# hibikid39/ndt_slam

Measured on AMD Instinct MI355X. Metric: scan-matches/sec (10k-pt scan vs 1M-pt NDT map), higher is better.
Workload: dtype f64

## Files before the change

ndt_slam_amd/csrc/ndt_map_build.hip.h:

```cpp


__device__ __forceinline__ unsigned f2ord(float f) {
  unsigned u = __float_as_uint(f);
  return (u & 0x80000000u) ? ~u : (u | 0x80000000u);
}
__host__ __device__ inline float ord2f(unsigned u) {
  u = (u & 0x80000000u) ? (u & 0x7fffffffu) : ~u;
  float f;
#if defined(__HIP_DEVICE_COMPILE__)
  f = __uint_as_float(u);
#else
  memcpy(&f, &u, 4);
#endif
  return f;
}

__global__ void __launch_bounds__(256)
map_minmax_kernel(const float *__restrict__ xy, size_t stride, size_t n, unsigned *__restrict__ bounds,
                  unsigned *__restrict__ out) {
  __shared__ float sh[4][4];
  float mnx = FLT_MAX, mny = FLT_MAX, mxx = -FLT_MAX, mxy = -FLT_MAX;
  const size_t step = (size_t)gridDim.x * blockDim.x;
  for (size_t i0 = blockIdx.x * (size_t)blockDim.x + threadIdx.x; i0 < n; i0 += 16 * step) {
    float2 p[16];
// ... 195 lines not shown
    for (int r = 0; r < 4; ++r) p[r] = e < n[r] ? load_pt(xy, stride, (size_t)mine[r]) : make_float2(0.f, 0.f);
#pragma unroll
    for (int r = 0; r < 4; ++r) {
      if (e >= n[r]) continue;
      int rank = 0;
      for (int j = 0; j < n[r]; j += 4) {
        const ndt_i4v q = *(const NDT_GLOBAL ndt_i4v_u *)(perm + s0[r] + j);
        rank += (q.x < mine[r]) ? 1 : 0;
        rank += (j + 1 < n[r] && q.y < mine[r]) ? 1 : 0;
        rank += (j + 2 < n[r] && q.z < mine[r]) ? 1 : 0;
        rank += (j + 3 < n[r] && q.w < mine[r]) ? 1 : 0;
      }
      pts[s0[r] + rank] = p[r];
    }
  }
}

constexpr int kBigWavesPerBlock = 4, kBigBlocks = 4096, kBigStage = 512;
constexpr int kBigRuns = 64;
__global__ void __launch_bounds__(256)
map_order_kernel(const int *__restrict__ start, size_t ng, unsigned small_blocks, const int *__restrict__ big,
                 const int *__restrict__ nbig, int big_cap, const int *__restrict__ perm, const float *__restrict__ xy,
                 size_t stride, float2 *__restrict__ pts) {
  __shared__ int stage[kBigWavesPerBlock][kBigStage];
  __shared__ int run_first[kBigWavesPerBlock][kBigRuns], run_pos[kBigWavesPerBlock][kBigRuns + 1];
  if (blockIdx.x < small_blocks) { order_small_voxels(blockIdx.x, start, ng, perm, xy, stride, pts); return; }
  const unsigned bblock = blockIdx.x - small_blocks, bblocks = gridDim.x - small_blocks;
  const int lane = threadIdx.x & 63, wv = threadIdx.x >> 6;
  const u64 lt = (1ull << lane) - 1ull;
  const int count = min(*nbig, big_cap);
  for (int q = bblock * kBigWavesPerBlock + wv; q < count; q += bblocks * kBigWavesPerBlock) {
    const int g = big[q];
    const int s0 = start[g], n = start[g + 1] - s0;
    const bool staged = n <= kBigStage;
    int nruns = 0;
    if (staged) {
      for (int e = lane; e < n; e += 64) stage[wv][e] = perm[s0 + e];
      __builtin_amdgcn_wave_barrier();
      for (int base = 0; base < n; base += 64) {
        const int e = base + lane;
        const int idx = e < n ? stage[wv][e] : 0, prev = (e > 0 && e < n) ? stage[wv][e - 1] : -2;
        const bool head = e < n && (e == 0 || idx != prev + 1);
        const u64 hm = __ballot(head);
        if (head) {
          const int r = nruns + __builtin_popcountll(hm & lt);
          if (r < kBigRuns) { run_first[wv][r] = idx; run_pos[wv][r] = e; }
        }
        nruns += __builtin_popcountll(hm);
      }
      if (lane == 0 && nruns <= kBigRuns) run_pos[wv][nruns] = n;
      __builtin_amdgcn_wave_barrier();
    }
    if (staged && nruns <= kBigRuns) {
      int seen = 0;
      for (int base = 0; base < n; base += 64) {
        const int e = base + lane;
        const int idx = e < n ? stage[wv][e] : 0, prev = (e > 0 && e < n) ? stage[wv][e - 1] : -2;
        const bool head = e < n && (e == 0 || idx != prev + 1);
        const u64 hm = __ballot(head);
        const int myrun = seen + __builtin_popcountll(hm & (lt | (1ull << lane))) - 1;
        seen += __builtin_popcountll(hm);
        if (e >= n) continue;
        const float2 p = load_pt(xy, stride, (size_t)idx);
        const int myfirst = run_first[wv][myrun], off = e - run_pos[wv][myrun];
        int dest = 0;
        for (int r = 0; r < nruns; ++r) {
          const int f = run_first[wv][r], len = run_pos[wv][r + 1] - run_pos[wv][r];
          dest += (f < myfirst) ? len : 0;
        }
        pts[s0 + dest + off] = p;
      }
      continue;
    }
    for (int e = lane; e < n; e += 64) {
      const int mine = staged ? stage[wv][e] : perm[s0 + e];
      int rank = 0;
      if (staged) { for (int j = 0; j < n; ++j) rank += (stage[wv][j] < mine) ? 1 : 0; }
      else        { for (int j = 0; j < n; ++j) rank += (perm[s0 + j] < mine) ? 1 : 0; }
      pts[s0 + rank] = load_pt(xy, stride, (size_t)mine);
    }
  }
}

struct LeafParams { int min_pts, cov_unbiased, cov_init_identity; double eig_mult; };

__device__ int leaf_finalize(const LeafParams &L, int n, double sx, double sy, double sxx,
                             double sxy, double syy, double szz, double mean[2], double icov[3]) {
  const double dn = (double)n;
  const double mx = sx / dn, my = sy / dn;
  mean[0] = mx; mean[1] = my;
  icov[0] = icov[1] = icov[2] = 0.0;
  double cxx, cxy, cyy, czz;
  if (!L.cov_unbiased) {
    cxx = (sxx - 2.0 * (sx * mx)) / dn + mx * mx;
    cxy = (sxy - 2.0 * (sy * mx)) / dn + my * mx;
    cyy = (syy - 2.0 * (sy * my)) / dn + my * my;
    czz = szz / dn;
    const double f = (dn - 1.0) / dn;
    cxx *= f; cxy *= f; cyy *= f; czz *= f;
  } else {
    cxx = (sxx - sx * mx) / (dn - 1.0);
    cxy = (sxy - sy * mx) / (dn - 1.0);
    cyy = (syy - sy * my) / (dn - 1.0);
    czz = szz / (dn - 1.0);
  }
  const double hd = 0.5 * (cxx - cyy), tr = 0.5 * (cxx + cyy);
  const double rad = sqrt(hd * hd + cxy * cxy);
  const double l1 = tr - rad, l2 = tr + rad;
  double vx, vy;
  if (rad == 0.0) { vx = 1.0; vy = 0.0; }
  else if (hd >= 0.0) { vx = hd + rad; vy = cxy; }
  else { vx = cxy; vy = rad - hd; }
  const double vn = sqrt(vx * vx + vy * vy);
  if (vn == 0.0) { vx = 1.0; vy = 0.0; } else { vx /= vn; vy /= vn; }
  double ev0, ev1, ev2; int k0, k1, k2;
  if (czz <= l1)      { ev0 = czz; k0 = 2; ev1 = l1; k1 = 0; ev2 = l2; k2 = 1; }
  else if (czz <= l2) { ev0 = l1; k0 = 0; ev1 = czz; k1 = 2; ev2 = l2; k2 = 1; }
  else                { ev0 = l1; k0 = 0; ev1 = l2; k1 = 1; ev2 = czz; k2 = 2; }
  if (ev0 < 0 || ev1 < 0 || ev2 <= 0) return 0;
  const double thr = L.eig_mult * ev2;
  bool rebuilt = false;
  if (ev0 < thr) { ev0 = thr; if (ev1 < thr) ev1 = thr; rebuilt = true; }
  double n1 = l1, n2 = l2;
  if (k0 == 0) n1 = ev0; else if (k0 == 1) n2 = ev0;
  if (k1 == 0) n1 = ev1; else if (k1 == 1) n2 = ev1;
  if (k2 == 0) n1 = ev2; else if (k2 == 1) n2 = ev2;
  if (rebuilt) {
    cxx = n1 * (vy * vy) + n2 * (vx * vx);
    cxy = -n1 * (vx * vy) + n2 * (vx * vy);
    cyy = n1 * (vx * vx) + n2 * (vy * vy);
  }
  const double det = cxx * cyy - cxy * cxy;
  icov[0] = cyy / det; icov[1] = -cxy / det; icov[2] = cxx / det;
  for (int a = 0; a < 3; ++a)
    if (icov[a] == (double)INFINITY || icov[a] == -(double)INFINITY) return -1;
  return 1;
}

__device__ __forceinline__ int write_voxel(const GridDims &G, const LeafParams &L, size_t g, int n, float fx, float fy,
                                           double sx, double sy, double sxx, double sxy, double syy, double szz,
                                           float2 *__restrict__ cent, double *__restrict__ rec, int *__restrict__ ) {
  if (n < L.min_pts) return 0;
  const int ix = (int)(g % G.div_x), iy = (int)(g / G.div_x);
  const size_t pg = (size_t)(iy + 2) * G.gw + (ix + 2);
  double mean[2], icov[3];
  const int ok = leaf_finalize(L, n, sx, sy, sxx, sxy, syy, szz, mean, icov);
  cent[pg] = make_float2(fx / (float)n, fy / (float)n);
  double *r = rec + pg * 8;
  r[0] = mean[0]; r[1] = mean[1]; r[2] = icov[0]; r[3] = icov[1]; r[4] = icov[2];
  r[5] = __longlong_as_double((long long)(((u64)__float_as_uint(fy / (float)n) << 32) | (u64)__float_as_uint(fx / (float)n)));
  return ok > 0 ? n : -n;
}

constexpr int kFinStage = 1536;
__global__ void __launch_bounds__(256)
map_finalize_kernel(GridDims G, LeafParams L,
                          const int *__restrict__ start,
                          const float2 *__restrict__ pts, float2 *__restrict__ cent, double *__restrict__ rec,
                          int *__restrict__ npts_grid, int *__restrict__ counters ,
                          unsigned *__restrict__ occ ,
                          u64 *__restrict__ tiles, int tiles_w ) {
  __shared__ float2 lp[4][kFinStage];
  const size_t ng = (size_t)G.div_x * G.div_y;
  size_t g = blockIdx.x * (size_t)blockDim.x + threadIdx.x;
  const bool live = g < ng;
  const int lane = threadIdx.x & 63, wv = threadIdx.x >> 6;
  int s0 = 0, s1 = 0;
  if (live) { s0 = start[g]; s1 = start[g + 1]; }
  const int n = s1 - s0;
  const int a = __shfl(s0, 0);
  int b = s1;
#pragma unroll
  for (int o = 1; o < 64; o <<= 1) b = max(b, __shfl_xor(b, o));
  const int m = b - a;
  const bool in_lds = m <= kFinStage;
  if (in_lds) {
    for (int j0 = 0; j0 < m; j0 += 8 * 64) {
      float2 t[8];
#pragma unroll
      for (int u = 0; u < 8; ++u) { const int j = j0 + u * 64 + lane; t[u] = pts[a + min(j, m - 1)]; }
#pragma unroll
      for (int u = 0; u < 8; ++u) { const int j = j0 + u * 64 + lane; if (j < m) lp[wv][j] = t[u]; }
    }
    __builtin_amdgcn_wave_barrier();
  }
  int flag = 0;
  if (n > 0) {
    float fx = 0.f, fy = 0.f;
    double sx = 0, sy = 0, sxx = 0, sxy = 0, syy = 0, szz = 0;
    if (L.cov_init_identity) { sxx = 1.0; syy = 1.0; szz = 1.0; }
    if (in_lds) {
      const float2 *q = &lp[wv][s0 - a];
      for (int s = 0; s < n; ++s) {
        const float2 p = q[s];
        fx += p.x; fy += p.y;
        const double X = (double)p.x, Y = (double)p.y;
        sx += X; sy += Y;
        sxx += X * X; sxy += X * Y; syy += Y * Y;
      }
    } else {
      float2 pb[8], pn[8];
#pragma unroll
      for (int u = 0; u < 8; ++u) pb[u] = pts[min(s0 + u, s1 - 1)];
      for (int s = s0; s < s1; s += 8) {
        if (s + 8 < s1) {
#pragma unroll
          for (int u = 0; u < 8; ++u) pn[u] = pts[min(s + 8 + u, s1 - 1)];
        }
#pragma unroll
        for (int u = 0; u < 8; ++u) {
          if (s + u >= s1) break;
          const float2 p = pb[u];
          fx += p.x; fy += p.y;
          const double X = (double)p.x, Y = (double)p.y;
          sx += X; sy += Y;
          sxx += X * X; sxy += X * Y; syy += Y * Y;
        }
#pragma unroll
        for (int u = 0; u < 8; ++u) pb[u] = pn[u];
      }
    }
    flag = write_voxel(G, L, g, n, fx, fy, sx, sy, sxx, sxy, syy, szz, cent, rec, counters);
    const int vy = (int)(g / (size_t)G.div_x), vx = (int)(g - (size_t)vy * G.div_x);
    atomicOr(tiles + (size_t)((vy >> 3) + 1) * tiles_w + (vx >> 3) + 1, 1ull << (8 * (vy & 7) + (vx & 7)));
  }
  if (live) npts_grid[g] = flag;
  const u64 in_set = __ballot(flag != 0);
  if ((threadIdx.x & 63) == 0 && live) {
    occ[g >> 5] = (unsigned)in_set;
    if ((g >> 5) + 1 < (ng + 31) / 32) occ[(g >> 5) + 1] = (unsigned)(in_set >> 32);
  }
}

__global__ void fill_f2_kernel(float2 *p, size_t n, float v, u64 *tiles, size_t ntiles) {
  for (size_t i = blockIdx.x * (size_t)blockDim.x + threadIdx.x; i < n; i += (size_t)gridDim.x * blockDim.x)
    p[i] = make_float2(v, v);
  for (size_t i = blockIdx.x * (size_t)blockDim.x + threadIdx.x; i < ntiles; i += (size_t)gridDim.x * blockDim.x)
    tiles[i] = 0ull;
}
```

ndt_slam_amd/csrc/ndt_mi355x.hip:

```cpp

#include <hip/hip_runtime.h>
#include <hip/hip_ext.h>

#include <algorithm>
#include <cfloat>
#include <cmath>
#include <cstdio>
#include <cstdlib>
#include <cstring>
#include <new>
#include <string>
#include <mutex>
#include <set>
#include <utility>
#include <vector>

#include "ndt_mi355x.h"

#pragma clang fp contract(off)

namespace {

thread_local std::string g_last_error;

#include "ndt_libm_f32.hip.h"
#include "ndt_common.hip.h"
#include "ndt_point.hip.h"
#include "ndt_optimizer.hip.h"
#include "ndt_fitness.hip.h"
#include "ndt_match.hip.h"
#include "ndt_map_build.hip.h"
#include "ndt_front.hip.h"
#include "ndt_localmap.hip.h"

}


struct ndt_ctx {
  int device = 0;
  hipStream_t stream = nullptr;
  hipStream_t own_stream = nullptr;
  hipEvent_t ev0 = nullptr, ev1 = nullptr;
  hipEvent_t evm0 = nullptr, evm1 = nullptr;
  hipEvent_t evb = nullptr;
  ndt_map *pending_map = nullptr;
  hipStream_t side = nullptr;
  hipEvent_t ev_fork = nullptr, ev_join = nullptr;
  bool map_ms_pending = false;
  unsigned *h_bounds = nullptr;
  std::string err;
  float map_ms = 0.f, align_ms = 0.f;
  void *d_scan = nullptr; size_t d_scan_cap = 0;
  void *d_off = nullptr; size_t d_off_cap = 0;
  void *d_init = nullptr; size_t d_init_cap = 0;
  void *d_res = nullptr; size_t d_res_cap = 0;
  void *d_tmp = nullptr; size_t d_tmp_cap = 0;
  void *d_trace = nullptr; size_t d_trace_cap = 0;
  void *d_rows = nullptr; size_t d_rows_cap = 0;
  void *d_sorted = nullptr; size_t d_sorted_cap = 0;
  void *d_sorted_x[2] = {nullptr, nullptr}; size_t d_sorted_x_cap[2] = {0, 0};
  void *d_fit = nullptr; size_t d_fit_cap = 0;
  void *d_fit_part = nullptr; size_t d_fit_part_cap = 0;
  void *d_far = nullptr; size_t d_far_cap = 0;
  void *d_ws = nullptr; size_t d_ws_cap = 0;
  void *d_ws_x[2] = {nullptr, nullptr}; size_t d_ws_x_cap[2] = {0, 0};
  void *d_pf = nullptr; size_t d_pf_cap = 0;
  void *d_rn = nullptr; size_t d_rn_cap = 0;
  void *d_mm = nullptr; size_t d_mm_cap = 0;
  void *h_mm = nullptr; size_t h_mm_cap = 0;
  hipEvent_t ev_mm = nullptr; bool mm_pending = false;
  int num_cus = 0;
  int helpers = -1;
  int workgroups = 0;
  int inject_fault = 0;
  struct PrepSet {
    void *sorted = nullptr; size_t sorted_cap = 0;
    void *recs = nullptr; size_t recs_cap = 0;
    void *maps = nullptr; size_t maps_cap = 0;
    hipEvent_t ev0 = nullptr, ready = nullptr;
    bool valid = false, timed = false;
    const void *scans = nullptr, *offsets = nullptr, *inits = nullptr, *map = nullptr;
    int B = 0, shared_scan = 0; size_t total_points = 0;
    int min_bx = 0, min_by = 0, div_x = 0, div_y = 0; float inv_leaf = 0.f;
    long long reader = -1;
  } prep[2];
  int prep_last = 1;
  float order_ms = 0.f;
  hipEvent_t ev_scratch = nullptr; hipStream_t scratch_stream = nullptr; bool scratch_used = false, scratch_recorded = false;
  size_t ws_clean = 0;
  size_t ws_clean_x[2] = {0, 0};
  static constexpr int kTimeRing = 64;
  hipEvent_t ev_ring[3 * kTimeRing] = {};
  int defer_fitness = 0;
  hipStream_t fit_stream = nullptr;
  bool ring_deferred[kTimeRing] = {};
  struct FitJob {
    MapView V; const float *scans = nullptr; const unsigned long long *offsets = nullptr; int B = 0, shared_scan = 0;
    size_t total_points = 0; float2 *sorted = nullptr; ndt_result *out = nullptr; unsigned char *ws = nullptr;
    size_t zero_bytes = 0, far_cnt_bytes = 0; bool sse = false; unsigned slot = 0;
  };
  bool deferred_pending = false;
  unsigned long long launches = 0;
};

struct ndt_map {
  ndt_ctx *ctx = nullptr;
  ndt_params prm;
  ndt_map_info info;
  bool info_valid = false;
  MapView view;
  size_t n = 0, ng = 0, npad = 0;
  int *count = nullptr, *start = nullptr, *npts_grid = nullptr;
  size_t count_cap = 0, start_cap = 0, npts_cap = 0;
  unsigned long long *scan_state = nullptr; size_t scan_state_cap = 0;
  unsigned scan_seq = 0;
  bool count_clean = false;
  int *perm = nullptr, *perm_sorted = nullptr; float2 *pts = nullptr;
  size_t perm_cap = 0, perm_sorted_cap = 0, pts_cap = 0;
  float2 *cent = nullptr; double *rec = nullptr; size_t cent_cap = 0, rec_cap = 0;
  unsigned *bounds = nullptr; int *counters = nullptr; int *total = nullptr;
  int *big = nullptr; size_t big_cap = 0;
  unsigned *occ = nullptr; size_t occ_cap = 0;
  unsigned long long *tiles = nullptr; size_t tiles_cap = 0;
  bool pending = false, pend_queued = false;
  const float *pend_xy = nullptr; size_t pend_stride = 0;
  GridDims grid; bool have_grid = false;
  void *d_xy_stage = nullptr; size_t d_xy_cap = 0;
  std::vector<std::pair<ndt_ctx *, unsigned long long>> readers;
};

namespace {

std::set<ndt_ctx *> g_live_ctx;
std::mutex g_live_mu;

int fail(ndt_ctx *ctx, int code, const std::string &msg) {
  g_last_error = msg;
  if (ctx) ctx->err = msg;
  return code;
}

#define HIP_TRY(ctx, expr)                                                                   \
  do {                                                                                       \
    hipError_t e_ = (expr);                                                                  \
    if (e_ != hipSuccess)                                                                    \
      return fail((ctx), NDT_E_HIP, std::string(#expr) + ": " + hipGetErrorString(e_));      \
  } while (0)

int ensure(ndt_ctx *ctx, void **p, size_t *cap, size_t need) {
  if (need <= *cap && *p) return NDT_OK;
  if (*p) { hipError_t e = hipFree(*p); (void)e; *p = nullptr; *cap = 0; }
  size_t want = need + need / 4 + 256;
  HIP_TRY(ctx, hipMalloc(p, want));
  *cap = want;
  return NDT_OK;
}

template <typename T>
int ensure_t(ndt_ctx *ctx, T **p, size_t *cap_elems, size_t need_elems) {
  size_t cap_bytes = *cap_elems * sizeof(T);
  void *vp = *p;
  int rc = ensure(ctx, &vp, &cap_bytes, need_elems * sizeof(T));
  *p = static_cast<T *>(vp);
  *cap_elems = cap_bytes / sizeof(T);
  return rc;
}

int scratch_begin(ndt_ctx *ctx, hipStream_t st, bool deferred_launch = false) {
  if (ctx->deferred_pending && !deferred_launch && ctx->launches > 0) {
    HIP_TRY(ctx, hipStreamWaitEvent(st, ctx->ev_ring[3 * ((ctx->launches - 1) % ndt_ctx::kTimeRing) + 2], 0));
    ctx->deferred_pending = false;
  }
  if (ctx->scratch_used && st != ctx->scratch_stream) {
    if (!ctx->scratch_recorded) HIP_TRY(ctx, hipEventRecord(ctx->ev_scratch, ctx->scratch_stream));
    HIP_TRY(ctx, hipStreamWaitEvent(st, ctx->ev_scratch, 0));
  }
  return NDT_OK;
}
int scratch_end(ndt_ctx *ctx, hipStream_t st) {
  ctx->scratch_recorded = false;
  if (st != ctx->stream) { HIP_TRY(ctx, hipEventRecord(ctx->ev_scratch, st)); ctx->scratch_recorded = true; }
  ctx->scratch_stream = st; ctx->scratch_used = true;
  return NDT_OK;
}

struct ScratchScope {
  ndt_ctx *ctx; hipStream_t st; bool open;
  ScratchScope(ndt_ctx *c, hipStream_t s) : ctx(c), st(s), open(true) {}
  ScratchScope(const ScratchScope &) = delete;
  ScratchScope &operator=(const ScratchScope &) = delete;
  int close() { open = false; return scratch_end(ctx, st); }
  ~ScratchScope() {
    if (!open) return;
    const std::string keep = ctx->err, keep_tl = g_last_error;
    (void)scratch_end(ctx, st);
    ctx->err = keep; g_last_error = keep_tl;
  }
};

OptParams opt_of(const ndt_params &p) {
// ... 73 lines not shown
#endif
constexpr int kDeferSets = NDT_DEFER_SETS;
static_assert(kDeferSets >= 2 && kDeferSets <= 3, "two spare sets of control words and ordered copies");
int launch_align(ndt_ctx *ctx, const ndt_map *map, hipStream_t st, const float *scans,
                 const unsigned long long *offsets, int B, int shared_scan, size_t total_points, const double *inits,
                 ndt_result *out, double *trace, int trace_cap, int *trace_rows, unsigned long long *prof,
                 ndt_ctx::PrepSet *pset = nullptr, bool defer = false) {
  const bool sse = map->prm.transform_sse != 0, incl = map->prm.radius_inclusive != 0;
  const int set = defer ? (int)(ctx->launches % (unsigned long long)kDeferSets) : 0;
  void **p_ws = set ? &ctx->d_ws_x[set - 1] : &ctx->d_ws; size_t *p_ws_cap = set ? &ctx->d_ws_x_cap[set - 1] : &ctx->d_ws_cap;
  size_t *p_clean = set ? &ctx->ws_clean_x[set - 1] : &ctx->ws_clean;
  void **p_sorted = set ? &ctx->d_sorted_x[set - 1] : &ctx->d_sorted; size_t *p_sorted_cap = set ? &ctx->d_sorted_x_cap[set - 1] : &ctx->d_sorted_cap;
  {
    const unsigned long long L = ctx->launches;
    auto end_of = [&](unsigned long long k) { return ctx->ev_ring[3 * (k % ndt_ctx::kTimeRing) + 2]; };
    if (!defer && L >= 1 && ctx->ring_deferred[(L - 1) % ndt_ctx::kTimeRing]) HIP_TRY(ctx, hipStreamWaitEvent(st, end_of(L - 1), 0));
    if (defer && L >= (unsigned long long)kDeferSets && ctx->ring_deferred[(L - kDeferSets) % ndt_ctx::kTimeRing]) HIP_TRY(ctx, hipStreamWaitEvent(st, end_of(L - kDeferSets), 0));
    if (defer && !ctx->fit_stream) HIP_TRY(ctx, hipStreamCreateWithFlags(&ctx->fit_stream, hipStreamNonBlocking));
  }
  const MapView &V = map->view;
  const OptParams O = opt_of(map->prm);
  const size_t zero_bytes = sizeof(WsHeader) + (size_t)B * sizeof(ScanCtl) + (size_t)B * kUnits * kUnitWords * sizeof(u64);
  const size_t ws_bytes = zero_bytes + (size_t)B * (kRegionCells / 8);
  const size_t ws_cap_before = *p_ws_cap;
  int rc = ensure(ctx, p_ws, p_ws_cap, ws_bytes);
  if (rc) return rc;
  if (*p_ws_cap != ws_cap_before) *p_clean = 0;
  const size_t slots = (shared_scan ? (size_t)B : (size_t)1) * total_points;
  if ((rc = ensure(ctx, p_sorted, p_sorted_cap, slots * sizeof(float2) + 16))) return rc;
  if (shared_scan && (rc = ensure(ctx, &ctx->d_fit, &ctx->d_fit_cap, slots * sizeof(float) + 16))) return rc;
  float2 *sorted = pset ? (float2 *)pset->sorted : (float2 *)*p_sorted;
  const PrepRec *prep = pset ? (const PrepRec *)pset->recs : nullptr;
  const unsigned *prep_map = pset ? (const unsigned *)pset->maps : nullptr;
  float *fit = (float *)ctx->d_fit;
  const size_t far_cnt_bytes = ((size_t)B * 2 * sizeof(unsigned) + 15) & ~(size_t)15;
  if (shared_scan && (rc = ensure(ctx, &ctx->d_far, &ctx->d_far_cap, far_cnt_bytes + slots * sizeof(unsigned) + 16))) return rc;
  if ((rc = ensure(ctx, &ctx->d_fit_part, &ctx->d_fit_part_cap, (slots / 64 + (size_t)B + 1) * sizeof(FitPart)))) return rc;
  FitPart *parts = (FitPart *)ctx->d_fit_part;
  if (*p_clean < zero_bytes) HIP_TRY(ctx, hipMemsetAsync(*p_ws, 0, zero_bytes, st));
  *p_clean = 0;
  unsigned char *ws = (unsigned char *)*p_ws;
  const int helpers = ctx->helpers >= 0 ? ctx->helpers : (B >= (ctx->workgroups > 0 ? ctx->workgroups : ctx->num_cus) ? kBatchHelpers : kDefaultHelpers);
  const int ncu = ctx->workgroups > 0 ? ctx->workgroups : ctx->num_cus;
  const int grid = helpers ? ncu : (B < ncu ? B : ncu);
  hipEvent_t *evr = ctx->ev_ring + 3 * (ctx->launches % ndt_ctx::kTimeRing);
  const bool chk = !(V.e_hi > 1.0 + 1e-6);
  ctx->ring_deferred[ctx->launches % ndt_ctx::kTimeRing] = defer;
#define NDT_LAUNCH(S_, I_, C_)                                                                                          \
  hipExtLaunchKernelGGL((ndt_align_kernel<S_, I_, C_>), dim3(grid), dim3(kBlock), 0, st, evr[0], evr[1], 0, V, O, scans, \
                        offsets, B, shared_scan, inits, out, trace, trace_cap, trace_rows, sorted, ws, helpers, prof, prep, prep_map)
  if (sse && incl)      NDT_LAUNCH(true, true, true);
  else if (sse && !chk) NDT_LAUNCH(true, false, false);
  else if (sse)         NDT_LAUNCH(true, false, true);
  else if (incl)        NDT_LAUNCH(false, true, true);
  else                  NDT_LAUNCH(false, false, true);
#undef NDT_LAUNCH
  auto entered = [&](int code) {
    if (code != NDT_OK) { hipError_t e = hipEventRecord(evr[2], st); (void)e; }
    {
      auto &rd = const_cast<ndt_map *>(map)->readers;
      std::lock_guard<std::mutex> lk(g_live_mu);
      bool found = false;
      for (auto &r : rd) if (r.first == ctx) { r.second = ctx->launches; found = true; }
      if (!found) rd.emplace_back(ctx, ctx->launches);
      if (pset) pset->reader = (long long)ctx->launches;
      ctx->launches++;
    }
    return code;
  };
  if (ctx->inject_fault > 0 && --ctx->inject_fault == 0)
    return entered(fail(ctx, NDT_E_HIP, "launch_align: injected fault behind the match kernel's dispatch (NDT_OPT_INJECT_FAULT)"));
  hipStream_t fs = st;
  if (defer) {
    fs = ctx->fit_stream;
    hipError_t e = hipStreamWaitEvent(fs, evr[1], 0);
    if (e != hipSuccess) return entered(fail(ctx, NDT_E_HIP, std::string("launch_align: hipStreamWaitEvent: ") + hipGetErrorString(e)));
  }
  {
    ndt_ctx::FitJob J;
    J.V = V; J.scans = scans; J.offsets = offsets; J.B = B; J.shared_scan = shared_scan; J.total_points = total_points;
    J.sorted = sorted; J.out = out; J.ws = ws; J.zero_bytes = zero_bytes; J.far_cnt_bytes = far_cnt_bytes; J.sse = sse;
    J.slot = (unsigned)(ctx->launches % ndt_ctx::kTimeRing);
    int qrc = queue_fitness(ctx, J, fs);
    if (qrc != NDT_OK) return entered(qrc);
  }
  {
    hipError_t e = hipGetLastError();
    if (e != hipSuccess) return entered(fail(ctx, NDT_E_HIP, std::string("launch_align: ") + hipGetErrorString(e)));
  }
  *p_clean = zero_bytes;
  if (defer) ctx->deferred_pending = true;
  return entered(NDT_OK);
}

int upload_exp_table(ndt_ctx *ctx) {
  double tab[64];
  for (int j = 0; j < 64; ++j) tab[j] = (double)exp2l((long double)j / 64.0L);
  HIP_TRY(ctx, hipMemcpyToSymbol(HIP_SYMBOL(c_exp2_tab), tab, sizeof(tab)));
  return NDT_OK;
}

}

extern "C" {

static void params_common(ndt_params *p) {
  memset(p, 0, sizeof(*p));
  p->resolution = 1.0f; p->step_size = 0.1; p->trans_eps = 0.01; p->max_iter = 35;
  p->outlier_ratio = 0.55; p->min_pts = 6; p->eig_mult = 0.01;
  p->conv_ge = 0; p->radius_inclusive = 0; p->stale_h_ang = 0;
  p->snap_thresh = 10e-5; p->mt_max_iter = 10; p->mt_mu = 1.e-4; p->mt_nu = 0.9; p->grid_margin = 0;
}

int ndt_params_pcl110(ndt_params *p) {
  if (!p) return NDT_E_ARG;
  params_common(p);
  p->cov_unbiased = 0; p->cov_init_identity = 1; p->transform_sse = 1; p->libm_f32 = 1;
  return NDT_OK;
}

int ndt_params_pcl18(ndt_params *p) {
  if (!p) return NDT_E_ARG;
  params_common(p);
  p->cov_unbiased = 0; p->cov_init_identity = 1; p->transform_sse = 0; p->libm_f32 = 0;
  return NDT_OK;
}

int ndt_params_pcl_new(ndt_params *p) {
  if (!p) return NDT_E_ARG;
  params_common(p);
  p->cov_unbiased = 1; p->cov_init_identity = 0; p->transform_sse = 1; p->libm_f32 = 1;
  return NDT_OK;
}

int ndt_default_params(ndt_params *p) { return ndt_params_pcl110(p); }

const char *ndt_last_error(const ndt_ctx *ctx) { return ctx ? ctx->err.c_str() : g_last_error.c_str(); }

static int ctx_init(ndt_ctx *c, int device) {
  c->device = device;
  HIP_TRY(c, hipSetDevice(device));
  HIP_TRY(c, hipStreamCreateWithFlags(&c->own_stream, hipStreamNonBlocking));
  c->stream = c->own_stream;
  HIP_TRY(c, hipEventCreate(&c->ev0));
  HIP_TRY(c, hipEventCreate(&c->ev1));
  HIP_TRY(c, hipEventCreate(&c->evm0));
  HIP_TRY(c, hipEventCreate(&c->evm1));
  HIP_TRY(c, hipEventCreateWithFlags(&c->evb, hipEventDisableTiming));
  {
    int lo = 0, hi = 0;
    HIP_TRY(c, hipDeviceGetStreamPriorityRange(&lo, &hi));
    HIP_TRY(c, hipStreamCreateWithPriority(&c->side, hipStreamNonBlocking, hi));
  }
  HIP_TRY(c, hipEventCreateWithFlags(&c->ev_fork, hipEventDisableTiming));
  HIP_TRY(c, hipEventCreateWithFlags(&c->ev_join, hipEventDisableTiming));
  HIP_TRY(c, hipEventCreateWithFlags(&c->ev_mm, hipEventDisableTiming));
  HIP_TRY(c, hipEventCreateWithFlags(&c->ev_scratch, hipEventDisableTiming));
  for (hipEvent_t &e : c->ev_ring) HIP_TRY(c, hipEventCreate(&e));
  HIP_TRY(c, hipHostMalloc((void **)&c->h_bounds, 64, hipHostMallocDefault));
  { int rc = upload_exp_table(c); if (rc) return rc; }
  hipDeviceProp_t prop;
  HIP_TRY(c, hipGetDeviceProperties(&prop, device));
  c->num_cus = prop.multiProcessorCount > 0 ? prop.multiProcessorCount : 1;
  c->helpers = -1;
  return NDT_OK;
}

int ndt_ctx_create(int device, ndt_ctx **out) {
  if (!out) return NDT_E_ARG;
  *out = nullptr;
  int ndev = 0;
  if (hipGetDeviceCount(&ndev) != hipSuccess || ndev <= 0)
    return fail(nullptr, NDT_E_NO_DEVICE, "no HIP device visible: libndt_mi355x has no CPU fallback");
  if (device < 0 || device >= ndev) return fail(nullptr, NDT_E_ARG, "device ordinal out of range");
  ndt_ctx *c = new (std::nothrow) ndt_ctx();
  if (!c) return NDT_E_NOMEM;
  const int rc = ctx_init(c, device);
  if (rc) { ndt_ctx_destroy(c); return rc; }
  { std::lock_guard<std::mutex> lk(g_live_mu); g_live_ctx.insert(c); }
  *out = c;
  return NDT_OK;
}

int ndt_ctx_set_option(ndt_ctx *c, int option, long long value) {
  if (!c) return NDT_E_ARG;
  switch (option) {
    case NDT_OPT_MAX_HELPERS:
      if (value < -1 || value > kMaxHelpers) return fail(c, NDT_E_ARG, "NDT_OPT_MAX_HELPERS: 0 .. 15, or -1 for the default");
      c->helpers = (int)value; return NDT_OK;
    case NDT_OPT_WORKGROUPS:
      if (value < 0 || value > c->num_cus) return fail(c, NDT_E_ARG, "NDT_OPT_WORKGROUPS: 0 (one per CU) .. number of CUs");
      c->workgroups = (int)value; return NDT_OK;
    case NDT_OPT_INJECT_FAULT:
      if (value < 0 || value > 1000000) return fail(c, NDT_E_ARG, "NDT_OPT_INJECT_FAULT: 0 (off) or the number of the launch that fails");
      c->inject_fault = (int)value; return NDT_OK;
    case NDT_OPT_DEFER_FITNESS:
      if (value != 0 && value != 1) return fail(c, NDT_E_ARG, "NDT_OPT_DEFER_FITNESS: 0 or 1");
      c->defer_fitness = (int)value; return NDT_OK;
    default: return fail(c, NDT_E_ARG, "ndt_ctx_set_option: unknown option");
  }
}

int ndt_ctx_destroy(ndt_ctx *c) {
  if (!c) return NDT_E_ARG;
  { std::lock_guard<std::mutex> lk(g_live_mu); g_live_ctx.erase(c); }
  hipError_t e;
  e = hipSetDevice(c->device);
  if (c->stream) e = hipStreamSynchronize(c->stream);
  if (c->fit_stream) { e = hipStreamSynchronize(c->fit_stream); e = hipStreamDestroy(c->fit_stream); }
  if (c->own_stream) e = hipStreamDestroy(c->own_stream);
  if (c->ev0) e = hipEventDestroy(c->ev0);
  if (c->ev1) e = hipEventDestroy(c->ev1);
  if (c->evm0) e = hipEventDestroy(c->evm0);
  if (c->evm1) e = hipEventDestroy(c->evm1);
  if (c->evb) e = hipEventDestroy(c->evb);
  if (c->side) { e = hipStreamSynchronize(c->side); e = hipStreamDestroy(c->side); }
  if (c->ev_fork) e = hipEventDestroy(c->ev_fork);
  if (c->ev_join) e = hipEventDestroy(c->ev_join);
  if (c->h_bounds) e = hipHostFree(c->h_bounds);
  if (c->ev_mm) e = hipEventDestroy(c->ev_mm);
  if (c->ev_scratch) e = hipEventDestroy(c->ev_scratch);
  for (hipEvent_t r : c->ev_ring) if (r) e = hipEventDestroy(r);
  for (ndt_ctx::PrepSet &S : c->prep) {
    if (S.ready && S.scans) e = hipEventSynchronize(S.ready);
    if (S.ev0) e = hipEventDestroy(S.ev0);
    if (S.ready) e = hipEventDestroy(S.ready);
    if (S.sorted) e = hipFree(S.sorted);
    if (S.recs) e = hipFree(S.recs);
    if (S.maps) e = hipFree(S.maps);
  }
  if (c->h_mm) e = hipHostFree(c->h_mm);
  void *bufs[] = {c->d_scan, c->d_off, c->d_init, c->d_res, c->d_tmp, c->d_trace, c->d_rows, c->d_sorted, c->d_sorted_x[0], c->d_sorted_x[1], c->d_ws_x[0], c->d_ws_x[1], c->d_fit, c->d_far, c->d_fit_part, c->d_ws, c->d_pf, c->d_rn, c->d_mm};
  for (void *b : bufs) if (b) e = hipFree(b);
  (void)e;
  delete c;
  return NDT_OK;
}

void *ndt_ctx_stream(ndt_ctx *c) { return c ? (void *)c->stream : nullptr; }

int ndt_ctx_set_stream(ndt_ctx *c, void *stream) {
  if (!c) return NDT_E_ARG;
  HIP_TRY(c, hipSetDevice(c->device));
  HIP_TRY(c, hipStreamSynchronize(c->stream));
  if (c->scratch_used && c->scratch_recorded) HIP_TRY(c, hipEventSynchronize(c->ev_scratch));
  c->scratch_used = false; c->scratch_recorded = false;
  c->stream = stream ? (hipStream_t)stream : c->own_stream;
  return NDT_OK;
}

int ndt_last_timing(const ndt_ctx *cc, float *map_ms, float *align_ms) {
  if (!cc) return NDT_E_ARG;
  ndt_ctx *c = const_cast<ndt_ctx *>(cc);
  if (c->map_ms_pending) {
    HIP_TRY(c, hipEventSynchronize(c->evm1));
    HIP_TRY(c, hipEventElapsedTime(&c->map_ms, c->evm0, c->evm1));
    c->map_ms_pending = false;
  }
  if (map_ms) *map_ms = c->map_ms;
  if (align_ms) *align_ms = c->align_ms;
  return NDT_OK;
}

int ndt_kernel_timing(ndt_ctx *c, int back, float *match_ms, float *fitness_ms) {
  if (!c || back < 0 || back >= ndt_ctx::kTimeRing || (unsigned long long)back >= c->launches)
    return fail(c, NDT_E_ARG, "ndt_kernel_timing: no such launch in the ring");
  hipEvent_t *evr = c->ev_ring + 3 * ((c->launches - 1 - (unsigned long long)back) % ndt_ctx::kTimeRing);
  HIP_TRY(c, hipEventSynchronize(evr[2]));
  float a = 0.f, f = 0.f;
  HIP_TRY(c, hipEventElapsedTime(&a, evr[0], evr[1]));
  HIP_TRY(c, hipEventElapsedTime(&f, evr[1], evr[2]));
  if (match_ms) *match_ms = a;
  if (fitness_ms) *fitness_ms = f;
  return NDT_OK;
}

int ndt_launch_interval(ndt_ctx *c, int back, float *interval_ms) {
  if (!c || !interval_ms || back < 0 || back + 1 >= ndt_ctx::kTimeRing || (unsigned long long)(back + 1) >= c->launches)
    return fail(c, NDT_E_ARG, "ndt_launch_interval: no such pair of launches in the ring");
  hipEvent_t *e1 = c->ev_ring + 3 * ((c->launches - 1 - (unsigned long long)back) % ndt_ctx::kTimeRing);
  hipEvent_t *e0 = c->ev_ring + 3 * ((c->launches - 2 - (unsigned long long)back) % ndt_ctx::kTimeRing);
  HIP_TRY(c, hipEventSynchronize(e1[0]));
  HIP_TRY(c, hipEventElapsedTime(interval_ms, e0[0], e1[0]));
  return NDT_OK;
}

int ndt_ctx_wait_launch(ndt_ctx *c, int back, void *stream) {
  if (!c || back < 0 || back >= ndt_ctx::kTimeRing || (unsigned long long)back >= c->launches)
    return fail(c, NDT_E_ARG, "ndt_ctx_wait_launch: no such launch in the ring");
  HIP_TRY(c, hipSetDevice(c->device));
  hipEvent_t *evr = c->ev_ring + 3 * ((c->launches - 1 - (unsigned long long)back) % ndt_ctx::kTimeRing);
  HIP_TRY(c, hipStreamWaitEvent(stream ? (hipStream_t)stream : c->stream, evr[2], 0));
  return NDT_OK;
}

int ndt_map_destroy(ndt_map *m) {
  if (!m) return NDT_E_ARG;
  hipError_t e = hipSetDevice(m->ctx->device);
  if (m->ctx->pending_map == m) {
    if (m->ctx->side) e = hipStreamSynchronize(m->ctx->side);
    m->ctx->pending_map = nullptr;
  }
  e = hipStreamSynchronize(m->ctx->stream);
  if (m->ctx->side) e = hipStreamSynchronize(m->ctx->side);
  void *bufs[] = {m->occ, m->tiles, m->big, m->count, m->start, m->scan_state, m->npts_grid, m->perm, m->perm_sorted, m->pts,
                  m->cent, m->rec, m->bounds, m->counters, m->total, m->d_xy_stage};
  for (void *b : bufs) if (b) e = hipFree(b);
  (void)e;
  delete m;
  return NDT_OK;
}

static int queue_build(ndt_ctx *ctx, ndt_map *m, const float *xy, size_t n, size_t stride, const ndt_params *prm,
                       const GridDims &G, bool requeue = false) {
  hipStream_t st = ctx->stream;
  const float inv_leaf = G.inv_leaf;
  const size_t ng = (size_t)G.div_x * G.div_y, npad = (size_t)G.gw * G.gh;
  m->ng = ng; m->npad = npad;
  const int tiles_w = (G.div_x + 7) / 8 + 2, tiles_h = (G.div_y + 7) / 8 + 2;
  const size_t ntile8 = (size_t)tiles_w * tiles_h;

  {
    int rc;
    const size_t ntiles_ = (ng + kScanTile - 1) / kScanTile;
    const size_t count_cap_before = m->count_cap;
    if ((rc = ensure_t(ctx, &m->count, &m->count_cap, ng + 1))) return rc;
    if (m->count_cap != count_cap_before) m->count_clean = false;
    if ((rc = ensure_t(ctx, &m->start, &m->start_cap, ng + 1 + 8))) return rc;
    if ((rc = ensure_t(ctx, &m->npts_grid, &m->npts_cap, ng + 1))) return rc;
    const size_t state_cap_before = m->scan_state_cap;
    if ((rc = ensure_t(ctx, &m->scan_state, &m->scan_state_cap, 2 * ntiles_ + 2))) return rc;
    if (m->scan_state_cap != state_cap_before)
      HIP_TRY(ctx, hipMemsetAsync(m->scan_state, 0, m->scan_state_cap * sizeof(unsigned long long), st));
    if ((rc = ensure_t(ctx, &m->perm, &m->perm_cap, n + 4))) return rc;
    if ((rc = ensure_t(ctx, &m->big, &m->big_cap, n / kBigVoxel + 1))) return rc;
    if ((rc = ensure_t(ctx, &m->occ, &m->occ_cap, (ng + 31) / 32 + 2))) return rc;
    if ((rc = ensure_t(ctx, &m->tiles, &m->tiles_cap, ntile8))) return rc;
    if ((rc = ensure_t(ctx, &m->pts, &m->pts_cap, n))) return rc;
    if ((rc = ensure_t(ctx, &m->cent, &m->cent_cap, npad))) return rc;
    if ((rc = ensure_t(ctx, &m->rec, &m->rec_cap, npad * 8))) return rc;
  }
  if (!m->count_clean) HIP_TRY(ctx, hipMemsetAsync(m->count, 0, m->count_cap * sizeof(int), st));
  m->count_clean = false;
  if (requeue) {
    HIP_TRY(ctx, hipEventRecord(ctx->ev_fork, st));
    HIP_TRY(ctx, hipStreamWaitEvent(ctx->side, ctx->ev_fork, 0));
  }
  fill_f2_kernel<<<grid_for(npad, 256), 256, 0, ctx->side>>>(m->cent, npad, INFINITY, m->tiles, ntile8);
  HIP_TRY(ctx, hipEventRecord(ctx->ev_join, ctx->side));

  map_count_kernel<<<grid_for(n, 256), 256, 0, st>>>(xy, stride, n, G, m->count, m->counters);
  const int ntiles = (int)((ng + kScanTile - 1) / kScanTile);
  int *const start = m->start + 4;
  const int big_cap = (int)(n / kBigVoxel + 1);
  m->scan_seq = (m->scan_seq + 1u) & 0x3fffffffu;
  if (m->scan_seq == 0u) m->scan_seq = 1u;
  scan_onepass_kernel<<<ntiles, kScanBlock, 0, st>>>(m->count, ng, m->scan_state, m->scan_seq, ntiles, m->counters + 3, start,
                                                     m->big, m->counters + 2, big_cap);
  map_scatter_kernel<<<grid_for(n, 256), 256, 0, st>>>(xy, stride, n, G, start, m->count, m->perm);
  HIP_TRY(ctx, hipGetLastError());
  m->count_clean = true;
  const unsigned small_blocks = (unsigned)((ng + kOrderVoxPerBlock - 1) / kOrderVoxPerBlock);
  map_order_kernel<<<small_blocks + kBigBlocks, 256, 0, st>>>(start, ng, small_blocks, m->big, m->counters + 2, big_cap, m->perm, xy, stride, m->pts);
  HIP_TRY(ctx, hipStreamWaitEvent(st, ctx->ev_join, 0));

  LeafParams L;
  L.min_pts = prm->min_pts; L.cov_unbiased = prm->cov_unbiased; L.cov_init_identity = prm->cov_init_identity;
  L.eig_mult = prm->eig_mult;
  hipExtLaunchKernelGGL(map_finalize_kernel, dim3((unsigned)((ng + 255) / 256)), dim3(256), 0, st, nullptr, ctx->evm1, 0, G, L, start,
                        m->pts, m->cent, m->rec, m->npts_grid, m->counters, m->occ, m->tiles, tiles_w);
  HIP_TRY(ctx, hipGetLastError());

  MapView &V = m->view;
  V.inv_leaf = inv_leaf; V.leaf = prm->resolution;
  V.r2 = (float)((double)prm->resolution * (double)prm->resolution);
  V.radius_inclusive = prm->radius_inclusive; V.transform_sse = prm->transform_sse;
  V.min_bx = G.min_bx; V.min_by = G.min_by; V.div_x = G.div_x; V.div_y = G.div_y; V.gw = G.gw; V.gh = G.gh;
  V.cent = m->cent; V.rec = m->rec; V.occ = m->occ; V.tiles = m->tiles; V.tiles_w = tiles_w; V.pt_start = start; V.pts = m->pts;
  gauss_constants(*prm, &V.d1, &V.d2);
  V.e_hi = pair_check_threshold(V.d2);
  m->info.min_bx = G.min_bx; m->info.min_by = G.min_by; m->info.div_x = G.div_x; m->info.div_y = G.div_y;
  m->info.n_points = n;
  return NDT_OK;
}

static int build_begin(ndt_ctx *ctx, ndt_map *m, const float *xy, size_t n, size_t stride, const ndt_params *prm) {
  hipStream_t st = ctx->stream;
  m->prm = *prm; m->n = n; m->info_valid = false;
  m->pend_xy = xy; m->pend_stride = stride; m->pend_queued = false;
  { std::lock_guard<std::mutex> lk(g_live_mu); m->readers.clear(); }
  HIP_TRY(ctx, hipEventRecord(ctx->evm0, st));
  HIP_TRY(ctx, hipStreamWaitEvent(ctx->side, ctx->evm0, 0));
  map_minmax_kernel<<<grid_for(n, 256 * 32, 128), 256, 0, ctx->side>>>(xy, stride, n, m->bounds, m->bounds + 4);
  HIP_TRY(ctx, hipMemcpyAsync(ctx->h_bounds, m->bounds + 4, 4 * sizeof(unsigned), hipMemcpyDeviceToHost, ctx->side));
  HIP_TRY(ctx, hipEventRecord(ctx->evb, ctx->side));
  const float inv_leaf = 1.0f / prm->resolution;
  if (m->have_grid && m->grid.inv_leaf == inv_leaf) {
    int rc = queue_build(ctx, m, xy, n, stride, prm, m->grid);
    if (rc) return rc;
    m->pend_queued = true;
  }
  m->pending = true;
  ctx->pending_map = m;
  return NDT_OK;
}

static int build_end(ndt_ctx *ctx, ndt_map *m) {
  hipStream_t st = ctx->stream;
  const ndt_params *prm = &m->prm;
  m->pending = false;
  ctx->pending_map = nullptr;
  const unsigned *hb = ctx->h_bounds;
  HIP_TRY(ctx, hipEventSynchronize(ctx->evb));
  if (hb[0] == 0xffffffffu) return fail(ctx, NDT_E_ARG, "ndt_map_build: no finite points");
  const float inv_leaf = 1.0f / prm->resolution;
  const float mnx = ord2f(hb[0]), mny = ord2f(hb[1]), mxx = ord2f(hb[2]), mxy = ord2f(hb[3]);
  GridDims G;
  G.inv_leaf = inv_leaf;
  auto vox = [&](float x) { return (int)fminf(fmaxf(floorf(x * inv_leaf), -1.0e9f), 1.0e9f); };
  G.min_bx = vox(mnx); G.min_by = vox(mny);
  long long dx = (long long)vox(mxx) - G.min_bx + 1;
  long long dy = (long long)vox(mxy) - G.min_by + 1;
  const int mg = prm->grid_margin > 0 ? (prm->grid_margin < 4096 ? prm->grid_margin : 4096) : 0;
  bool same = false;
  if (m->pend_queued) {
    const GridDims &S = m->grid;
    const long long lo_x = (long long)G.min_bx - S.min_bx, lo_y = (long long)G.min_by - S.min_by;
    const long long hi_x = ((long long)S.min_bx + S.div_x) - ((long long)G.min_bx + dx);
    const long long hi_y = ((long long)S.min_by + S.div_y) - ((long long)G.min_by + dy);
    same = lo_x >= 0 && lo_y >= 0 && hi_x >= 0 && hi_y >= 0 && lo_x <= 2 * mg && lo_y <= 2 * mg && hi_x <= 2 * mg && hi_y <= 2 * mg;
  }
  if (same) G = m->grid;
  else {
    G.min_bx -= mg; G.min_by -= mg; dx += 2 * mg; dy += 2 * mg;
    if (dx > (1LL << 28) || dy > (1LL << 28) || dx * dy > (1LL << 28))
      return fail(ctx, NDT_E_GRID, "ndt_map_build: voxel grid larger than 2^28 cells");
    G.div_x = (int)dx; G.div_y = (int)dy; G.gw = G.div_x + 4; G.gh = G.div_y + 4;
  }
  int redone = 0;
  if (!same) {
    if (m->pend_queued) {
      {
        std::lock_guard<std::mutex> lk(g_live_mu);
        for (auto &r : m->readers) {
          ndt_ctx *rc_ = r.first;
          if (g_live_ctx.count(rc_) == 0 || rc_->launches <= r.second) continue;
          const bool wrapped = rc_->launches - 1 - r.second >= (unsigned long long)ndt_ctx::kTimeRing;
          const unsigned long long which = wrapped ? rc_->launches - 1 : r.second;
          hipEvent_t *evr = rc_->ev_ring + 3 * (which % ndt_ctx::kTimeRing);
          HIP_TRY(ctx, hipStreamWaitEvent(st, evr[2], 0));
        }
      }
    }
    int rc = queue_build(ctx, m, m->pend_xy, m->n, m->pend_stride, prm, G, m->pend_queued);
    if (rc) return rc;
    redone = m->pend_queued ? 1 : 0;
  }
  m->grid = G; m->have_grid = true;
  ctx->map_ms_pending = true;
  return redone;
}

static int map_build_impl(ndt_ctx *ctx, ndt_map *m, const float *xy, size_t n, size_t stride, const ndt_params *prm) {
  if (ctx->pending_map) return fail(ctx, NDT_E_ARG, "ndt_map_build: ndt_map_rebuild_end is still owed for a map of this context");
  int rc = build_begin(ctx, m, xy, n, stride, prm);
  if (rc) { m->pending = false; ctx->pending_map = nullptr; return rc; }
  rc = build_end(ctx, m);
  return rc < 0 ? rc : NDT_OK;
}

int ndt_map_build_dev(ndt_ctx *ctx, const float *xy, size_t n, size_t stride, const ndt_params *prm,
                      ndt_map **pmap) {
  if (!ctx) return fail(nullptr, NDT_E_ARG, "null context");
  if (!xy || n == 0 || !prm || !pmap || !(prm->resolution > 0) || stride < 8 || (stride & 7))
    return fail(ctx, NDT_E_ARG, "ndt_map_build: bad arguments (need n > 0, resolution > 0, stride % 8 == 0)");
  if (n > (size_t)INT32_MAX) return fail(ctx, NDT_E_ARG, "ndt_map_build: more than 2^31 points");
  if (*pmap && (*pmap)->ctx != ctx) return fail(ctx, NDT_E_ARG, "ndt_map_build: the map belongs to another context");
  HIP_TRY(ctx, hipSetDevice(ctx->device));
  ndt_map *m = *pmap;
  const bool fresh = (m == nullptr);
  if (fresh) {
    m = new (std::nothrow) ndt_map();
    if (!m) return NDT_E_NOMEM;
    m->ctx = ctx;
    hipError_t e = hipMalloc(&m->bounds, 16 * sizeof(unsigned));
    const unsigned init_b[16] = {0xffffffffu, 0xffffffffu, 0u, 0u};
    if (e == hipSuccess) e = hipMemcpy(m->bounds, init_b, sizeof(init_b), hipMemcpyHostToDevice);
    if (e == hipSuccess) e = hipMalloc(&m->counters, 4 * sizeof(int));
    if (e == hipSuccess) e = hipMalloc(&m->total, sizeof(int));
    if (e != hipSuccess) { ndt_map_destroy(m); return fail(ctx, NDT_E_HIP, std::string("ndt_map_build: hipMalloc: ") + hipGetErrorString(e)); }
  }
  const int rc = map_build_impl(ctx, m, xy, n, stride, prm);
  if (rc) {
    m->have_grid = false;
    if (fresh) ndt_map_destroy(m);
    return rc;
  }
  *pmap = m;
  return NDT_OK;
}


int ndt_map_rebuild_begin(ndt_ctx *ctx, const float *xy, size_t n, size_t stride, const ndt_params *prm, ndt_map *m) {
  if (!ctx) return fail(nullptr, NDT_E_ARG, "null context");
  if (!xy || n == 0 || !prm || !m || !(prm->resolution > 0) || stride < 8 || (stride & 7) || n > (size_t)INT32_MAX)
    return fail(ctx, NDT_E_ARG, "ndt_map_rebuild_begin: bad arguments");
  if (m->ctx != ctx) return fail(ctx, NDT_E_ARG, "ndt_map_rebuild_begin: the map belongs to another context");
  if (ctx->pending_map) return fail(ctx, NDT_E_ARG, "ndt_map_rebuild_begin: ndt_map_rebuild_end is still owed for a map of this context");
  if (!m->have_grid || m->grid.inv_leaf != 1.0f / prm->resolution)
    return fail(ctx, NDT_E_ARG, "ndt_map_rebuild_begin: the map has no earlier build at this resolution (use ndt_map_build_dev)");
  HIP_TRY(ctx, hipSetDevice(ctx->device));
  const int rc = build_begin(ctx, m, xy, n, stride, prm);
  if (rc) { m->have_grid = false; m->pending = false; ctx->pending_map = nullptr; }
  return rc;
}

int ndt_map_rebuild_end(ndt_ctx *ctx, ndt_map *m) {
  if (!ctx) return fail(nullptr, NDT_E_ARG, "null context");
  if (!m || m->ctx != ctx || !m->pending || ctx->pending_map != m)
    return fail(ctx, NDT_E_ARG, "ndt_map_rebuild_end: no ndt_map_rebuild_begin is open for this map");
  HIP_TRY(ctx, hipSetDevice(ctx->device));
  const int rc = build_end(ctx, m);
  if (rc < 0) m->have_grid = false;
  return rc;
}

int ndt_map_build(ndt_ctx *ctx, const float *xy_host, size_t n, size_t stride, const ndt_params *prm,
                  ndt_map **pmap) {
  if (!ctx) return fail(nullptr, NDT_E_ARG, "null context");
  if (!xy_host || n == 0 || !pmap || stride < 8 || (stride & 7)) return fail(ctx, NDT_E_ARG, "ndt_map_build: bad arguments");
  HIP_TRY(ctx, hipSetDevice(ctx->device));
  void *stage = nullptr; size_t cap = 0;
  if (*pmap) { stage = (*pmap)->d_xy_stage; cap = (*pmap)->d_xy_cap; }
  int rc = ensure(ctx, &stage, &cap, n * stride);
  if (rc) return rc;
  HIP_TRY(ctx, hipMemcpyAsync(stage, xy_host, n * stride, hipMemcpyHostToDevice, ctx->stream));
  rc = ndt_map_build_dev(ctx, (const float *)stage, n, stride, prm, pmap);
  if (rc == NDT_OK) { hipError_t e = hipStreamSynchronize(ctx->stream); if (e != hipSuccess) rc = fail(ctx, NDT_E_HIP, hipGetErrorString(e)); }
  if (*pmap) { (*pmap)->d_xy_stage = stage; (*pmap)->d_xy_cap = cap; }
  else { hipError_t e = hipFree(stage); (void)e; }
  return rc;
}

// ... 785 lines not shown
```

Measured before the change: 652,100.

## Fold centroid/tile border fill into finalize kernel, drop side-stream fill

Removes the separate fill_f2 kernel on the side stream, which set every centroid to infinity and zeroed the occupancy tiles, along with its fork/join events. Instead, finalize writes infinity only for empty or undersized voxels, and extra blocks appended to the finalize launch fill the padding border and build the tile bitmasks directly from the start offsets instead of using atomicOr. This cuts a full-grid memset-like pass and its cross-stream synchronisation. It also adds waits on reader events in build_begin, which now handle the hazard the fork event used to cover.

```diff
diff --git a/ndt_slam_amd/csrc/ndt_map_build.hip.h b/ndt_slam_amd/csrc/ndt_map_build.hip.h
--- a/ndt_slam_amd/csrc/ndt_map_build.hip.h
+++ b/ndt_slam_amd/csrc/ndt_map_build.hip.h
@@ -371,6 +371,42 @@
   return ok > 0 ? n : -n;
 }
 
+__device__ __forceinline__ void voxel_borders(unsigned block, const GridDims &G, const int *__restrict__ start,
+                                              float2 *__restrict__ cent, u64 *__restrict__ tiles, int tiles_w, int tiles_h) {
+  const size_t t = (size_t)block * 256 + threadIdx.x;
+  const size_t ntile8 = (size_t)tiles_w * tiles_h;
+  if (t < 8 * ntile8) {
+    const size_t w = t >> 3;
+    const int r = (int)(t & 7);
+    const int tx = (int)(w % (size_t)tiles_w), ty = (int)(w / (size_t)tiles_w);
+    const int x0 = (tx - 1) * 8, y = (ty - 1) * 8 + r;
+    u64 word = 0;
+    if (tx >= 1 && ty >= 1 && y < G.div_y) {
+      const int *row = start + (size_t)y * G.div_x;
+      int o[9];
+#pragma unroll
+      for (int c = 0; c < 9; ++c) o[c] = row[min(x0 + c, G.div_x)];
+      unsigned byte = 0;
+#pragma unroll
+      for (int c = 0; c < 8; ++c) byte |= (x0 + c < G.div_x && o[c + 1] > o[c]) ? 1u << c : 0u;
+      word = (u64)byte << (8 * r);
+    }
+#pragma unroll
+    for (int k = 1; k < 8; k <<= 1) word |= __shfl_xor(word, k);
+    if (r == 0) tiles[w] = word;
+    return;
+  }
+  const size_t k = t - 8 * ntile8, ring = 4 * (size_t)G.gw;
+  size_t y, x;
+  if (k < ring) { const size_t rr = k / G.gw; y = rr < 2 ? rr : G.gh - 4 + rr; x = k % G.gw; }
+  else {
+    const size_t k2 = k - ring;
+    if (k2 >= 4 * (size_t)G.div_y) return;
+    const size_t c = k2 & 3; y = 2 + k2 / 4; x = c < 2 ? c : G.gw - 4 + c;
+  }
+  cent[y * G.gw + x] = make_float2(INFINITY, INFINITY);
+}
+
 constexpr int kFinStage = 1536;
 __global__ void __launch_bounds__(256)
 map_finalize_kernel(GridDims G, LeafParams L,
@@ -378,8 +414,10 @@
                           const float2 *__restrict__ pts, float2 *__restrict__ cent, double *__restrict__ rec,
                           int *__restrict__ npts_grid, int *__restrict__ counters ,
                           unsigned *__restrict__ occ ,
-                          u64 *__restrict__ tiles, int tiles_w ) {
+                          u64 *__restrict__ tiles, int tiles_w ,
+                          int tiles_h, unsigned vox_blocks) {
   __shared__ float2 lp[4][kFinStage];
+  if (blockIdx.x >= vox_blocks) { voxel_borders(blockIdx.x - vox_blocks, G, start, cent, tiles, tiles_w, tiles_h); return; }
   const size_t ng = (size_t)G.div_x * G.div_y;
   size_t g = blockIdx.x * (size_t)blockDim.x + threadIdx.x;
   const bool live = g < ng;
@@ -440,20 +478,17 @@
       }
     }
     flag = write_voxel(G, L, g, n, fx, fy, sx, sy, sxx, sxy, syy, szz, cent, rec, counters);
-    const int vy = (int)(g / (size_t)G.div_x), vx = (int)(g - (size_t)vy * G.div_x);
-    atomicOr(tiles + (size_t)((vy >> 3) + 1) * tiles_w + (vx >> 3) + 1, 1ull << (8 * (vy & 7) + (vx & 7)));
-  }
-  if (live) npts_grid[g] = flag;
+  }
+  if (live) {
+    if (n <= 0 || n < L.min_pts) {
+      const int ix = (int)(g % G.div_x), iy = (int)(g / G.div_x);
+      cent[(size_t)(iy + 2) * G.gw + (ix + 2)] = make_float2(INFINITY, INFINITY);
+    }
+    npts_grid[g] = flag;
+  }
   const u64 in_set = __ballot(flag != 0);
   if ((threadIdx.x & 63) == 0 && live) {
     occ[g >> 5] = (unsigned)in_set;
     if ((g >> 5) + 1 < (ng + 31) / 32) occ[(g >> 5) + 1] = (unsigned)(in_set >> 32);
   }
 }
-
-__global__ void fill_f2_kernel(float2 *p, size_t n, float v, u64 *tiles, size_t ntiles) {
-  for (size_t i = blockIdx.x * (size_t)blockDim.x + threadIdx.x; i < n; i += (size_t)gridDim.x * blockDim.x)
-    p[i] = make_float2(v, v);
-  for (size_t i = blockIdx.x * (size_t)blockDim.x + threadIdx.x; i < ntiles; i += (size_t)gridDim.x * blockDim.x)
-    tiles[i] = 0ull;
-}
diff --git a/ndt_slam_amd/csrc/ndt_mi355x.hip b/ndt_slam_amd/csrc/ndt_mi355x.hip
--- a/ndt_slam_amd/csrc/ndt_mi355x.hip
+++ b/ndt_slam_amd/csrc/ndt_mi355x.hip
@@ -45,7 +45,6 @@
   hipEvent_t evb = nullptr;
   ndt_map *pending_map = nullptr;
   hipStream_t side = nullptr;
-  hipEvent_t ev_fork = nullptr, ev_join = nullptr;
   bool map_ms_pending = false;
   unsigned *h_bounds = nullptr;
   std::string err;
@@ -425,8 +424,6 @@
     HIP_TRY(c, hipDeviceGetStreamPriorityRange(&lo, &hi));
     HIP_TRY(c, hipStreamCreateWithPriority(&c->side, hipStreamNonBlocking, hi));
   }
-  HIP_TRY(c, hipEventCreateWithFlags(&c->ev_fork, hipEventDisableTiming));
-  HIP_TRY(c, hipEventCreateWithFlags(&c->ev_join, hipEventDisableTiming));
   HIP_TRY(c, hipEventCreateWithFlags(&c->ev_mm, hipEventDisableTiming));
   HIP_TRY(c, hipEventCreateWithFlags(&c->ev_scratch, hipEventDisableTiming));
   for (hipEvent_t &e : c->ev_ring) HIP_TRY(c, hipEventCreate(&e));
@@ -488,8 +485,6 @@
   if (c->evm1) e = hipEventDestroy(c->evm1);
   if (c->evb) e = hipEventDestroy(c->evb);
   if (c->side) { e = hipStreamSynchronize(c->side); e = hipStreamDestroy(c->side); }
-  if (c->ev_fork) e = hipEventDestroy(c->ev_fork);
-  if (c->ev_join) e = hipEventDestroy(c->ev_join);
   if (c->h_bounds) e = hipHostFree(c->h_bounds);
   if (c->ev_mm) e = hipEventDestroy(c->ev_mm);
   if (c->ev_scratch) e = hipEventDestroy(c->ev_scratch);
@@ -615,12 +610,7 @@
   }
   if (!m->count_clean) HIP_TRY(ctx, hipMemsetAsync(m->count, 0, m->count_cap * sizeof(int), st));
   m->count_clean = false;
-  if (requeue) {
-    HIP_TRY(ctx, hipEventRecord(ctx->ev_fork, st));
-    HIP_TRY(ctx, hipStreamWaitEvent(ctx->side, ctx->ev_fork, 0));
-  }
-  fill_f2_kernel<<<grid_for(npad, 256), 256, 0, ctx->side>>>(m->cent, npad, INFINITY, m->tiles, ntile8);
-  HIP_TRY(ctx, hipEventRecord(ctx->ev_join, ctx->side));
+  (void)requeue;
 
   map_count_kernel<<<grid_for(n, 256), 256, 0, st>>>(xy, stride, n, G, m->count, m->counters);
   const int ntiles = (int)((ng + kScanTile - 1) / kScanTile);
@@ -635,13 +625,15 @@
   m->count_clean = true;
   const unsigned small_blocks = (unsigned)((ng + kOrderVoxPerBlock - 1) / kOrderVoxPerBlock);
   map_order_kernel<<<small_blocks + kBigBlocks, 256, 0, st>>>(start, ng, small_blocks, m->big, m->counters + 2, big_cap, m->perm, xy, stride, m->pts);
-  HIP_TRY(ctx, hipStreamWaitEvent(st, ctx->ev_join, 0));
 
   LeafParams L;
   L.min_pts = prm->min_pts; L.cov_unbiased = prm->cov_unbiased; L.cov_init_identity = prm->cov_init_identity;
   L.eig_mult = prm->eig_mult;
-  hipExtLaunchKernelGGL(map_finalize_kernel, dim3((unsigned)((ng + 255) / 256)), dim3(256), 0, st, nullptr, ctx->evm1, 0, G, L, start,
-                        m->pts, m->cent, m->rec, m->npts_grid, m->counters, m->occ, m->tiles, tiles_w);
+  const unsigned vox_blocks = (unsigned)((ng + 255) / 256);
+  const size_t nborder = 4 * (size_t)G.gw + 4 * (size_t)G.div_y;
+  const unsigned edge_blocks = (unsigned)((8 * ntile8 + nborder + 255) / 256);
+  hipExtLaunchKernelGGL(map_finalize_kernel, dim3(vox_blocks + edge_blocks), dim3(256), 0, st, nullptr, ctx->evm1, 0, G, L, start,
+                        m->pts, m->cent, m->rec, m->npts_grid, m->counters, m->occ, m->tiles, tiles_w, tiles_h, vox_blocks);
   HIP_TRY(ctx, hipGetLastError());
 
   MapView &V = m->view;
@@ -661,7 +653,18 @@
   hipStream_t st = ctx->stream;
   m->prm = *prm; m->n = n; m->info_valid = false;
   m->pend_xy = xy; m->pend_stride = stride; m->pend_queued = false;
-  { std::lock_guard<std::mutex> lk(g_live_mu); m->readers.clear(); }
+  {
+    std::lock_guard<std::mutex> lk(g_live_mu);
+    for (auto &r : m->readers) {
+      ndt_ctx *rc_ = r.first;
+      if (g_live_ctx.count(rc_) == 0 || rc_->launches <= r.second) continue;
+      const bool wrapped = rc_->launches - 1 - r.second >= (unsigned long long)ndt_ctx::kTimeRing;
+      const unsigned long long which = wrapped ? rc_->launches - 1 : r.second;
+      if (!wrapped && !rc_->ring_deferred[which % ndt_ctx::kTimeRing]) continue;
+      HIP_TRY(ctx, hipStreamWaitEvent(st, rc_->ev_ring[3 * (which % ndt_ctx::kTimeRing) + 2], 0));
+    }
+    m->readers.clear();
+  }
   HIP_TRY(ctx, hipEventRecord(ctx->evm0, st));
   HIP_TRY(ctx, hipStreamWaitEvent(ctx->side, ctx->evm0, 0));
   map_minmax_kernel<<<grid_for(n, 256 * 32, 128), 256, 0, ctx->side>>>(xy, stride, n, m->bounds, m->bounds + 4);
```

Result: no change. 654,800 (median of 6 runs) (+0.4%).
